# dimfeld/perceive

Hardware: AMD Instinct MI355X
Metric: vectors scanned/sec (exact cosine top-10, 384-d f32, batch=64) (higher is better)
Workload: dtype f32

## Files before the change

### include/perceive_hip.h

```cpp
#ifndef PERCEIVE_HIP_H
#define PERCEIVE_HIP_H

#include <stddef.h>
#include <stdint.h>

#ifdef __cplusplus
extern "C" {
#endif

typedef int pcv_status;
enum {
    PCV_OK = 0,
    PCV_ERR_INVALID = 1,
    PCV_ERR_DEVICE = 2,
    PCV_ERR_UNSUPPORTED = 3,
    PCV_ERR_IO = 4,
    PCV_ERR_INTERNAL = 5
};

enum { PCV_METRIC_COSINE = 0, PCV_METRIC_DOT = 1 };

typedef struct pcv_ctx pcv_ctx;
typedef struct pcv_searcher pcv_searcher;
typedef struct pcv_model pcv_model;
// ... 125 lines not shown
pcv_status pcv_comm_destroy(pcv_comm* c);
pcv_status pcv_searcher_search_sharded(pcv_searcher* s, pcv_comm* c, const float* queries, int n_queries,
                                       const int64_t* source_ids, int n_sources, int k, int64_t* out_ids,
                                       float* out_scores, int* out_counts);
pcv_status pcv_searcher_search_sharded_dq(pcv_searcher* s, pcv_comm* c, const void* d_queries, int n_queries,
                                          const int64_t* source_ids, int n_sources, int k, int64_t* out_ids,
                                          float* out_scores, int* out_counts);
pcv_status pcv_comm_all_gather(pcv_comm* c, const void* d_send, void* d_recv, size_t bytes_per_rank);

pcv_status pcv_dot_product(pcv_ctx* ctx, const float* a, int B, const float* m, int64_t N, int dim,
                           float* out);
pcv_status pcv_cosine_similarity(pcv_ctx* ctx, const float* a, int B, const float* m, int64_t N, int dim,
                                 float* out);

typedef struct pcv_scan_stats {
    int64_t rows_scanned;
    int64_t bytes_algorithmic;
    float scan_ms;
    float total_ms;
    int64_t candidates;
    int32_t scan_launches;
    int32_t overflow_reruns;
    int32_t kernel_used;
    int32_t screening_copy;
    float host_enqueue_ms;
    float host_wait_ms;
    int64_t bytes_streamed;
    int32_t speculation_reruns;
    int32_t mid_copy;
    int64_t coarse_survivors;
    int64_t mid_survivors;
    int64_t narrow_survivors;
    int32_t screen_bits;
} pcv_scan_stats;
pcv_status pcv_searcher_last_stats(pcv_searcher* s, pcv_scan_stats* out);


typedef struct pcv_model_desc {
    int32_t vocab_size;
    int32_t hidden;
    int32_t layers;
    int32_t heads;
    int32_t intermediate;
    int32_t max_positions;
    int32_t type_vocab;
    float layer_norm_eps;
    int32_t pooling;
    int32_t normalize;
    int32_t dense_out;
    int32_t dense_activation;
    int32_t max_seq_length;
    int32_t compute;
    int32_t embedding_size;
    int32_t shared_layers;
    int32_t hidden_act;
} pcv_model_desc;
enum { PCV_GELU_ERF = 0, PCV_GELU_TANH = 1 };
enum { PCV_POOL_MEAN = 0, PCV_POOL_CLS = 1, PCV_POOL_MAX = 2, PCV_POOL_MEAN_SQRT_LEN = 3 };
enum { PCV_ACT_IDENTITY = 0, PCV_ACT_TANH = 1 };
enum { PCV_COMPUTE_F32 = 0, PCV_COMPUTE_BF16X3 = 1, PCV_COMPUTE_F16X2 = 2 };

void pcv_model_desc_minilm_l6(pcv_model_desc* d);

pcv_status pcv_model_create(pcv_ctx* ctx, const pcv_model_desc* desc, const char* weights_path,
                            uint64_t synthetic_seed, pcv_model** out);
pcv_status pcv_model_destroy(pcv_model* m);
// ... 57 lines not shown
```

### perceive_amd/_ffi.py

```python
import ctypes as C
import os

_HERE = os.path.dirname(os.path.abspath(__file__))
LIB_PATH = os.path.join(_HERE, "libperceive_hip.so")

PCV_OK = 0
METRIC_COSINE, METRIC_DOT = 0, 1
KERNEL_AUTO, KERNEL_WAVE, KERNEL_MFMA = 0, 1, 2
POOL_MEAN, POOL_CLS, POOL_MAX, POOL_MEAN_SQRT_LEN = 0, 1, 2, 3
ACT_IDENTITY, ACT_TANH = 0, 1
COMPUTE_F32, COMPUTE_BF16X3, COMPUTE_F16X2 = 0, 1, 2


class PcvError(RuntimeError):
    def __init__(self, status, message):
        super().__init__(f"perceive_hip status {status}: {message}")
        self.status = status


class Hit(C.Structure):
    _fields_ = [("score", C.c_double), ("pos", C.c_int64), ("id", C.c_int64)]


class ScanStats(C.Structure):
    _fields_ = [
        ("rows_scanned", C.c_int64),
        ("bytes_algorithmic", C.c_int64),
        ("scan_ms", C.c_float),
        ("total_ms", C.c_float),
        ("candidates", C.c_int64),
        ("scan_launches", C.c_int32),
        ("overflow_reruns", C.c_int32),
        ("kernel_used", C.c_int32),
        ("screening_copy", C.c_int32),
        ("host_enqueue_ms", C.c_float),
        ("host_wait_ms", C.c_float),
        ("bytes_streamed", C.c_int64),
        ("speculation_reruns", C.c_int32),
        ("mid_copy", C.c_int32),
        ("coarse_survivors", C.c_int64),
        ("mid_survivors", C.c_int64),
        ("narrow_survivors", C.c_int64),
        ("screen_bits", C.c_int32),
    ]


class ModelDesc(C.Structure):
    _fields_ = [
        ("vocab_size", C.c_int32),
        ("hidden", C.c_int32),
        ("layers", C.c_int32),
        ("heads", C.c_int32),
        ("intermediate", C.c_int32),
        ("max_positions", C.c_int32),
        ("type_vocab", C.c_int32),
        ("layer_norm_eps", C.c_float),
        ("pooling", C.c_int32),
        ("normalize", C.c_int32),
        ("dense_out", C.c_int32),
        ("dense_activation", C.c_int32),
        ("max_seq_length", C.c_int32),
        ("compute", C.c_int32),
        ("embedding_size", C.c_int32),
        ("shared_layers", C.c_int32),
        ("hidden_act", C.c_int32),
    ]


class EncodeStats(C.Structure):
    _fields_ = [("total_ms", C.c_float), ("flops", C.c_double), ("batch", C.c_int32), ("seq_len", C.c_int32)]


_P = C.c_void_p
_I64P = C.c_void_p
_F32P = C.c_void_p
_U8P = C.c_void_p
# ... 145 lines not shown
```

### perceive_amd/csrc/scan.h

```cpp
#pragma once
#include <hip/hip_runtime.h>
#include <stdint.h>

#include "../../include/perceive_hip.h"

namespace pcv {

constexpr int kBlockRows = 32;
constexpr int kMaxK = PCV_MAX_RESULTS;
constexpr int kSeedPartRows = 256;
constexpr int kSeedParts = 64;
constexpr int kMaxWaveQueries = 4;
constexpr int kHot = 256;
constexpr int kMfmaQueries = 256;
constexpr int kScale8Stride = 1;

struct SegDesc {
    const float4* blk;
    const float* scale;
    const int64_t* ids;
    int64_t id0;
    int64_t pos0;
    uint32_t nrows;
    uint32_t nblocks;
    uint32_t blk0;
    uint32_t pad;
    const uint4* blk16;
    const uint4* blk8;
    const uint4* mid16;
    const float* scale16;
    const float* scale8;
    const uint4* blk6;
    const float4* scale6;
};
constexpr uint32_t kFlagSix = 1u << 31;
constexpr uint32_t kTuneNoSix = 1u << 29;
constexpr uint32_t kTuneForceSix = 1u << 31;

struct pcv_hit_dev {
    double score;
    int64_t pos;
    int64_t id;
};

struct CeilRec {
    double score;
    int64_t pos;
    float lo, hi;
};

struct ScanParams {
    const SegDesc* seg;
    int nseg;
    uint32_t total_blocks;
    int D;
    int D4;
    int B;
    int k;
    int metric;
    uint32_t tile_rows;
    const CeilRec* ceil;
    const float* queries;
    float* qf32;
    uint16_t* qbf16;
    int8_t* q8;
    float* q8c;
    float* qraw;
    float* margin;
    float* margin32;
    uint32_t* tau;
// ... 105 lines not shown
```

### perceive_amd/csrc/scan_kernels.hip

```cpp
#include <algorithm>
#include <cstdlib>
#include <numeric>
#include <type_traits>

#include "common.h"
#include "scan.h"
#include "synth.h"

#ifndef PCV_EXP
#define PCV_EXP 0
#endif
namespace pcv {
namespace {

typedef __bf16 bf16x8 __attribute__((ext_vector_type(8)));
typedef float f32x8 __attribute__((ext_vector_type(8)));
typedef float f32x16 __attribute__((ext_vector_type(16)));
typedef float f32x4 __attribute__((ext_vector_type(4)));

#define PCV_GLOBAL __attribute__((address_space(1)))
template <class T>
__device__ __forceinline__ T gld(const T* p) {
    return *(const PCV_GLOBAL T*)p;
}
// ... 304 lines not shown
        const float s_blk = !any_row ? __builtin_nanf("") : (bm > 0.0f ? 127.0f / bm : 1.0f);
        for (int g = h; g < D16; g += 2) {
            uint32_t w[4] = {0, 0, 0, 0};
#pragma unroll
            for (int e = 0; e < 4; ++e)
                if (searchable && 4 * g + e < D4) {
                    const float4 v = src[(size_t)(4 * g + e) * 32];
                    const float y[4] = {v.x * sc, v.y * sc, v.z * sc, v.w * sc};
#pragma unroll
                    for (int j = 0; j < 4; ++j) {
                        const int qv = max(-127, min(127, (int)rintf(y[j] * s_blk)));
                        w[e] |= (uint32_t)(qv & 0xff) << (8 * j);
                    }
                }
            blk8[((size_t)b * D16 + g) * 32 + r] = make_uint4(w[0], w[1], w[2], w[3]);
        }
        if (lane == 0) scale8[b] = s_blk;
    }
}


__global__ __launch_bounds__(256) void pack6_kernel(const float4* __restrict__ blk, const float* __restrict__ scale,
                                                    const uint4* __restrict__ blk8, const float* __restrict__ scale8,
                                                    const uint32_t* __restrict__ blocks, uint4* __restrict__ blk6,
                                                    float4* __restrict__ scale6, uint32_t first_block, uint32_t nblocks, int D4) {
    const int lane = threadIdx.x & 63, r = lane & 31, h = lane >> 5;
    const int D16 = ((D4 * 4 + 127) & ~127) >> 4, NCH = D16 >> 3;
    for (uint32_t i = (blocks ? 0u : first_block) + blockIdx.x * 4 + (threadIdx.x >> 6); i < nblocks; i += gridDim.x * 4) {
        const uint32_t b = blocks ? blocks[i] : i;
        const float sc = scale[(size_t)b * 32 + r];
        const float s = scale8[b];
        const bool searchable = sc != 0.0f && s == s;
        const double inv_s = searchable ? 1.0 / (double)s : 0.0;
        double e2 = 0.0, n2 = 0.0;
        for (int ch = 0; ch < NCH; ++ch) {
            uint32_t w[16];
#pragma unroll
            for (int ks = 0; ks < 4; ++ks) {
                const int f16 = ch * 8 + 2 * ks + h;
                const uint4 v = blk8[((size_t)b * D16 + f16) * 32 + r];
                w[4 * ks] = v.x;
                w[4 * ks + 1] = v.y;
                w[4 * ks + 2] = v.z;
                w[4 * ks + 3] = v.w;
#pragma unroll
                for (int e = 0; e < 4; ++e) {
                    const int f4 = 4 * f16 + e;
                    if (!searchable || f4 >= D4) continue;
                    const float4 x = blk[((size_t)b * D4 + f4) * 32 + r];
                    const float y[4] = {x.x * sc, x.y * sc, x.z * sc, x.w * sc};
                    const uint32_t word = w[4 * ks + e];
#pragma unroll
                    for (int j = 0; j < 4; ++j) {
                        const int x8 = (int)(int8_t)(word >> (8 * j));
                        const double xt = (double)(4 * (x8 >> 2)) * inv_s + 1.5 * inv_s;
                        const double d = (double)y[j] - xt;
                        e2 += d * d;
                        n2 += xt * xt;
                    }
                }
            }
            uint32_t u[16];
#pragma unroll
            for (int d = 0; d < 16; ++d) {
                const uint32_t biased = w[d] ^ 0x80808080u;
                u[d] = (biased >> 2) & 0x3f3f3f3fu;
            }
            uint32_t lo[8], hi[4];
#pragma unroll
            for (int k = 0; k < 8; ++k) lo[k] = (u[2 * k] & 0x0f0f0f0fu) | ((u[2 * k + 1] & 0x0f0f0f0fu) << 4);
#pragma unroll
            for (int k = 0; k < 4; ++k) {
                hi[k] = 0;
#pragma unroll
                for (int m = 0; m < 4; ++m) hi[k] |= ((u[4 * k + m] >> 4) & 0x03030303u) << (2 * m);
            }
            uint4* dst = blk6 + ((size_t)b * NCH + ch) * 3 * 64 + lane;
            dst[0] = make_uint4(lo[0], lo[1], lo[2], lo[3]);
            dst[64] = make_uint4(lo[4], lo[5], lo[6], lo[7]);
            dst[128] = make_uint4(hi[0], hi[1], hi[2], hi[3]);
        }
        e2 += __shfl_xor(e2, 32);
        n2 += __shfl_xor(n2, 32);
#pragma unroll
        for (int off = 16; off > 0; off >>= 1) {
            e2 = fmax(e2, __shfl_xor(e2, off));
            n2 = fmax(n2, __shfl_xor(n2, off));
        }
        if (lane == 0) {
            const float up = 1.0f + 0x1p-19f;
            const bool any = s == s;
            scale6[b] = make_float4(s, any ? (float)(sqrt(e2) * (double)s) * up : 0.0f, any ? (float)(sqrt(n2) * (double)s) * up : 0.0f, 0.0f);
        }
    }
}


__global__ __launch_bounds__(256) void mid_pack_kernel(const float4* __restrict__ blk, const float* __restrict__ scale, uint4* __restrict__ mid16,
                                                       float* __restrict__ scale16, uint32_t first_row, uint32_t nrows, int D4) {
    const int lane = threadIdx.x & 63;
    const int P8 = D4 >> 1;
    for (uint32_t row = first_row + blockIdx.x * 4 + (threadIdx.x >> 6); row < nrows; row += gridDim.x * 4) {
        const float sc = scale[row];
        const float4* src = blk + (size_t)(row >> 5) * D4 * 32 + (row & 31);
        float mx = 0.0f;
        for (int j = lane; j < P8; j += 64) {
            const float4 a = src[(size_t)(2 * j) * 32], b = src[(size_t)(2 * j + 1) * 32];
            mx = fmaxf(mx, fmaxf(fmaxf(fmaxf(fabsf(a.x * sc), fabsf(a.y * sc)), fmaxf(fabsf(a.z * sc), fabsf(a.w * sc))),
                                 fmaxf(fmaxf(fabsf(b.x * sc), fabsf(b.y * sc)), fmaxf(fabsf(b.z * sc), fabsf(b.w * sc)))));
        }
#pragma unroll
        for (int off = 32; off > 0; off >>= 1) mx = fmaxf(mx, __shfl_xor(mx, off));
        const bool searchable = sc != 0.0f && mx < __builtin_inff();
        const float s2 = !searchable ? 0.0f : (mx > 0.0f ? 32766.0f / mx : 1.0f);
        for (int j = lane; j < P8; j += 64) {
            const float4 a = src[(size_t)(2 * j) * 32], b = src[(size_t)(2 * j + 1) * 32];
            const float y[8] = {a.x * sc, a.y * sc, a.z * sc, a.w * sc, b.x * sc, b.y * sc, b.z * sc, b.w * sc};
            uint32_t w[4];
#pragma unroll
            for (int e = 0; e < 4; ++e) {
                const int lo = searchable ? max(-32767, min(32767, (int)rintf(y[2 * e] * s2))) : 0;
                const int hi = searchable ? max(-32767, min(32767, (int)rintf(y[2 * e + 1] * s2))) : 0;
                w[e] = ((uint32_t)lo & 0xffffu) | ((uint32_t)hi << 16);
            }
            mid16[(size_t)row * P8 + j] = make_uint4(w[0], w[1], w[2], w[3]);
// ... 524 lines not shown
    const int64_t i = t / D4src;
    const int f4 = (int)(t % D4src);
    if (i >= n) return;
    const int64_t gp = pos[i];
    int s = -1;
    for (int j = 0; j < nseg; ++j)
        if (gp >= segs[j].pos0 && gp < segs[j].pos0 + (int64_t)segs[j].nrows) s = j;
    float4 v = make_float4(__builtin_nanf(""), __builtin_nanf(""), __builtin_nanf(""), __builtin_nanf(""));
    int64_t id = -1;
    if (s >= 0) {
        const uint32_t row = (uint32_t)(gp - segs[s].pos0);
        v = segs[s].blk[((size_t)(row >> 5) * D4 + f4) * 32 + (row & 31)];
        id = segs[s].ids ? segs[s].ids[row] : segs[s].id0 + row;
    }
    const float vv[4] = {v.x, v.y, v.z, v.w};
    for (int j = 0; j < 4; ++j)
        if (f4 * 4 + j < D) out_rows[i * D + f4 * 4 + j] = vv[j];
    if (f4 == 0 && out_ids) out_ids[i] = id;
}


__global__ __launch_bounds__(256) void reset_scan_state_kernel(uint32_t* __restrict__ tau, uint32_t* __restrict__ slots,
                                                               uint32_t* __restrict__ cand_cnt) {
    const int t = blockIdx.x * 256 + threadIdx.x;
    if (t < kMfmaQueries * kMaxK) slots[t] = kKeyNegInf;
    if (t < kMfmaQueries) {
        tau[t * kHot] = kKeyNegInf;
        tau[kMfmaQueries * kHot + t] = kKeyNegInf;
        cand_cnt[t * kHot] = 0;
        cand_cnt[t * kHot + 32] = 0;
        cand_cnt[t * kHot + 33] = 0;
        cand_cnt[t * kHot + 34] = 0;
    }
}

__device__ __forceinline__ bool is_seed_block(const ScanParams& p, int si, uint32_t lb) {
    return si == 0 && (lb & ((1u << p.seed_shift) - 1u)) == 0 && (lb >> p.seed_shift) < p.seed_blocks;
}

__device__ __forceinline__ uint32_t seed_threshold_key(const ScanParams& p, int q, int sub ) {
    uint32_t mn = 0xffffffffu;
    if (q < p.B)
        for (int j = sub; j < p.k; j += 4) mn = min(mn, ld_relaxed(&p.slots[(size_t)q * kMaxK + j]));
    mn = min(mn, (uint32_t)__shfl_xor(mn, 1));
    mn = min(mn, (uint32_t)__shfl_xor(mn, 2));
    return q < p.B ? mn : kKeyNegInf;
}

__global__ __launch_bounds__(256) void upload_kernel(const uint4* __restrict__ src_pinned, uint4* __restrict__ dst, uint32_t n16) {
    const uint32_t i = blockIdx.x * 256 + threadIdx.x;
    if (i < n16) dst[i] = src_pinned[i];
}

template <int QG>
__global__ __launch_bounds__(256) void prep_seed_kernel(const ScanParams* __restrict__ pp, const float4* __restrict__ seg0_blk,
                                                        const float* __restrict__ seg0_scale, uint32_t nseed) {
    const ScanParams& p = *pp;
    extern __shared__ __attribute__((aligned(16))) float smem[];
    const int Dp = p.D4 * 4, D = p.D;
    float* sq = smem;
    uint32_t* gmax = (uint32_t*)(smem + QG * Dp);
    const int part = blockIdx.x, q0 = blockIdx.y * QG, tid = threadIdx.x;
    const bool writer = part == 0;
    static_assert(kSeedPartRows == 256, "one seed row per thread");
    const uint32_t sr = part * kSeedPartRows + tid;
    const uint32_t row = (((sr >> 5) << p.seed_shift) << 5) | (sr & 31);
// ... 736 lines not shown
    float sblk[kRing];
    uint32_t tail, head, done, pad;
};
__device__ __forceinline__ uint32_t lds_ld(const uint32_t* p) { return __hip_atomic_load(p, __ATOMIC_RELAXED, __HIP_MEMORY_SCOPE_WORKGROUP); }
__device__ __forceinline__ void lds_st(uint32_t* p, uint32_t v) { __hip_atomic_store(p, v, __ATOMIC_RELAXED, __HIP_MEMORY_SCOPE_WORKGROUP); }
__device__ __forceinline__ uint32_t lds_add(uint32_t* p, uint32_t v) {
    return __hip_atomic_fetch_add(p, v, __ATOMIC_RELAXED, __HIP_MEMORY_SCOPE_WORKGROUP);
}
#define PCV_LDS_ORDER() asm volatile("" ::: "memory")

template <bool SIX = false>
__device__ __forceinline__ void ring_push(SurvRing& ring, uint32_t m, const i32x16& acc, float sblk, uint32_t q, uint32_t hh, uint32_t si,
                                          uint32_t elb, float off = 0.0f) {
    const uint32_t n = (uint32_t)__builtin_popcount(m);
    uint32_t pos = 0;
    if (m) pos = lds_add(&ring.tail, n);
    while (__any(m != 0 && (pos + n - 1u) - lds_ld(&ring.head) >= kRing)) __builtin_amdgcn_s_sleep(2);
    const uint32_t hib = 0x80000000u | (si << 13) | (q << 5) | (4u * hh);
#pragma unroll
    for (int i = 0; i < 16; ++i) {
        if (m & (1u << i)) {
            const uint32_t slot = pos & (kRing - 1);
            lds_st(&ring.lo[slot], elb);
            ring.acc[slot] = SIX ? __builtin_bit_cast(int, fmaf(4.0f, (float)acc[i], off)) : acc[i];
            ring.sblk[slot] = sblk;
            PCV_LDS_ORDER();
            lds_st(&ring.hi[slot], hib + (uint32_t)((i & 3) + 8 * (i >> 2)));
            ++pos;
        }
    }
}

constexpr uint32_t kStack = 2048;
struct DrainStack {
    uint32_t lo[kStack], hi[kStack];
    int acc[kStack];
    float sblk[kStack];
};
constexpr int kSixMaxDp8 = 384;
constexpr int kSixPieces = kSixMaxDp8 / 16 / 8;
template <int NQ, bool SIX = false>
__device__ __forceinline__ void drain_survivors(const ScanParams& p, SurvRing& ring, DrainStack& stk, const uint32_t* ltau0, const float* lsq,
                                                const float* lvq, float* lU, int lane, int D4, uint32_t streaming, unsigned long long* stamp,
                                                const uint4* lq8 = nullptr, int LDQ = 0, float* lT6 = nullptr) {
    static_assert(NQ <= 64, "one query per lane");
#ifdef PCV_STAMPS
#define PCV_DSTAMP(slot) if (stamp && lane == 0) stamp[slot] = __builtin_amdgcn_s_memrealtime();
#define PCV_DCOUNT(slot, n) if (stamp && lane == 0) stamp[slot] += (n);
#define PCV_DMAX(hi, lo_) if (stamp && lane == 0) { const unsigned long long o = stamp[2]; \
        stamp[2] = (max(o >> 32, (unsigned long long)(hi)) << 32) | max(o & 0xffffffffull, (unsigned long long)(lo_)); }
#else
#define PCV_DSTAMP(slot)
#define PCV_DCOUNT(slot, n)
#define PCV_DMAX(hi, lo_)
#endif
    PCV_DSTAMP(0)
#ifdef PCV_STAMPS
    const unsigned long long clk0 = __builtin_amdgcn_s_memtime();
#endif
    const int Dp = D4 * 4, Dp8 = (Dp + 127) & ~127;
    const uint32_t g = (uint32_t)lane >> 3;
    const int sub = lane & 7;
    const int ql = lane < NQ ? lane : NQ - 1;
    const float my_sq = lsq[ql], my_vq = lvq[ql];
    const uint32_t my_tau0 = ltau0[ql];
    const float my_e32 = ql < p.B ? 0.5f * gld(&p.margin32[ql]) : 0.0f;
    const float nrm = (p.metric == PCV_METRIC_DOT) ? p.max_norm : 1.0f;
    const float c1 = 0.5002f * sqrtf((float)Dp8) * nrm;
    const float dead = (p.metric == PCV_METRIC_DOT) ? -__builtin_inff() : __builtin_inff();
    uint32_t my_tau = ld_relaxed(&p.tau_c[ql]);
    uint32_t head = 0, sp = 0, idle = 0;
    int c_si = -1;
    const float4* c_blk = nullptr;
    const float* c_scale = nullptr;
    const uint4* c_mid = nullptr;
    const float* c_s16 = nullptr;
    __builtin_amdgcn_s_setprio(3);

    auto work = [&](bool on, uint32_t hi, uint32_t lo) {
#ifdef PCV_STAMPS
        const unsigned long long ts = __builtin_amdgcn_s_memrealtime();
#endif
        const int q = (int)((hi >> 5) & 0xffu), rib = (int)(hi & 31u), si = (int)((hi >> 13) & ((1u << kRingSegBits) - 1u));
        const uint32_t lb = lo, row = lb * 32u + (uint32_t)rib;
        if (on && si != c_si) {
            c_si = si;
            c_blk = gld(&p.seg[si].blk);
            c_scale = gld(&p.seg[si].scale);
            c_mid = gld(&p.seg[si].mid16);
            c_s16 = gld(&p.seg[si].scale16);
        }
        float sc = 0.0f, m32 = 0.0f, s2 = 1.0f, l1 = 0.0f, part = 0.0f;
        uint32_t tkey = kKeyNegInf;
        const bool has_mid = on && c_mid != nullptr;
        const float* qf = p.qf32 + (size_t)q * Dp;
        if (on) {
            sc = gld(&c_scale[row]);
// ... 102 lines not shown
            first = false;
            int src = -1;
#pragma unroll
            for (uint32_t j = 0; j < 8; ++j) {
                if (set) {
                    const int s0 = __builtin_ctzll(set);
                    set &= set - 1;
                    if (g == j) src = s0;
                }
            }
            const bool on = src >= 0;
            work(on, (uint32_t)__shfl((int)ehi, on ? src : 0), (uint32_t)__shfl((int)elo, on ? src : 0));
        }
    };

    for (;;) {
        refresh((idle & 7u) == 0);

        uint32_t tail = lds_ld(&ring.tail);
        bool over = false;
        if (tail == head) {
            over = lds_ld(&ring.done) == streaming;
            if (over) {
                PCV_LDS_ORDER();
                tail = lds_ld(&ring.tail);
            }
        }
        if (tail != head) {
            idle = 0;
            const uint32_t n = min(tail - head, 64u);
            bool have = (uint32_t)lane < n;
            uint32_t ehi = 0, elo = 0;
            int eacc = 0;
            float esb = 0.0f;
            if (have) {
                const uint32_t slot = (head + (uint32_t)lane) & (kRing - 1);
                do ehi = lds_ld(&ring.hi[slot]);
                while (!(ehi & 0x80000000u));
                PCV_LDS_ORDER();
                elo = lds_ld(&ring.lo[slot]);
                eacc = ring.acc[slot];
                esb = ring.sblk[slot];
                PCV_LDS_ORDER();
                lds_st(&ring.hi[slot], 0u);
            }
            head += n;
            PCV_LDS_ORDER();
            if (lane == 0) lds_st(&ring.head, head);
            const int eq = (int)((ehi >> 5) & 0xffu);
            if constexpr (SIX) {
                if (have) g_atomic_add(&p.cand_cnt[eq * kHot + 34], 1u);
                have = have && __builtin_bit_cast(float, eacc) >= esb * __shfl(myT6, eq);
                const int P16 = ((D4 * 4 + 127) & ~127) >> 4;
                unsigned long long set = __ballot(have);
                while (set) {
                    const unsigned long long taken_from = set;
                    int src = -1;
#pragma unroll
                    for (uint32_t j = 0; j < 8; ++j) {
                        if (set) {
                            const int s0 = __builtin_ctzll(set);
                            set &= set - 1;
                            if (g == j) src = s0;
                        }
                    }
                    const unsigned long long taken = taken_from & ~set;
                    const bool on = src >= 0;
                    const uint32_t hi8 = (uint32_t)__shfl((int)ehi, on ? src : 0), lb8 = (uint32_t)__shfl((int)elo, on ? src : 0);
                    const int q8q = (int)((hi8 >> 5) & 0xffu), rib = (int)(hi8 & 31u), si8 = (int)((hi8 >> 13) & ((1u << kRingSegBits) - 1u));
                    int part = 0;
                    float sb = 0.0f;
                    if (on) {
                        const uint4* b8 = gld(&p.seg[si8].blk8);
                        sb = gld(gld(&p.seg[si8].scale8) + lb8);
                        uint4 v[kSixPieces];
#pragma unroll
                        for (int j = 0; j < kSixPieces; ++j)
                            if (sub + 8 * j < P16) v[j] = __builtin_bit_cast(uint4, gld4((const float4*)b8 + ((size_t)lb8 * P16 + sub + 8 * j) * 32 + rib));
#pragma unroll
                        for (int j = 0; j < kSixPieces; ++j)
                            if (sub + 8 * j < P16) {
                                const uint4 qv = lq8[(size_t)q8q * LDQ + sub + 8 * j];
                                part = __builtin_amdgcn_sdot4((int)v[j].x, (int)qv.x, part, false);
                                part = __builtin_amdgcn_sdot4((int)v[j].y, (int)qv.y, part, false);
                                part = __builtin_amdgcn_sdot4((int)v[j].z, (int)qv.z, part, false);
                                part = __builtin_amdgcn_sdot4((int)v[j].w, (int)qv.w, part, false);
                            }
                    }
#pragma unroll
                    for (int off = 4; off > 0; off >>= 1) part += __shfl_xor(part, off);
                    const int rank = (int)__builtin_popcountll(taken & ((1ull << lane) - 1ull));
                    const int a8 = __shfl(part, 8 * rank);
                    const float s8 = __shfl(sb, 8 * rank);
                    if ((taken >> lane) & 1ull) {
                        eacc = a8;
                        esb = s8;
                    }
                }
            }
            const float U = __shfl(myU, eq), vq = __shfl(my_vq, eq), Tq = __shfl(myT, eq);
            const float rhs = fmaf(esb, U, -vq);
            const bool keep = have && (float)eacc >= rhs;
            const bool likely = keep && (float)eacc >= fmaf(0.25f, rhs, 0.75f * esb * Tq);
            if (SIX ? keep : have) g_atomic_add(&p.cand_cnt[eq * kHot + 32], 1u);
            const unsigned long long wait = __ballot(keep && !likely);
            const uint32_t nw = (uint32_t)__builtin_popcountll(wait);
            PCV_DCOUNT(4, n)
            PCV_DCOUNT(7, n - (uint32_t)__builtin_popcountll(__ballot(keep)))
            PCV_DMAX(tail - (head - n), sp + nw)
            if (sp + nw <= kStack) {
                if (keep && !likely) {
                    const uint32_t at = sp + (uint32_t)__builtin_popcountll(wait & ((1ull << lane) - 1ull));
                    stk.lo[at] = elo;
                    stk.hi[at] = ehi;
                    stk.acc[at] = eacc;
                    stk.sblk[at] = esb;
                }
                sp += nw;
                work_set(__ballot(likely), ehi, elo);
            } else {
                work_set(__ballot(keep), ehi, elo);
            }
        } else if (sp > 0) {
            idle = 0;
            const uint32_t n = min(sp, 8u);
            sp -= n;
            const bool have = g < n;
            const uint32_t at = sp + (have ? g : 0u);
            const uint32_t ehi = stk.hi[at], elo = stk.lo[at];
            const int eacc = stk.acc[at];
            const float esb = stk.sblk[at];
            const int eq = (int)((ehi >> 5) & 0xffu);
            const float U = __shfl(myU, eq), vq = __shfl(my_vq, eq);
            const bool keep = have && (float)eacc >= fmaf(esb, U, -vq);
            PCV_DCOUNT(7, n - (uint32_t)__builtin_popcountll(__ballot(keep && sub == 0)))
            if (__any(keep)) work(keep, ehi, elo);
        } else if (over) {
            break;
        } else {
            ++idle;
            __builtin_amdgcn_s_sleep(4);
        }
    }
    PCV_DSTAMP(3)
    PCV_DCOUNT(1, __builtin_amdgcn_s_memtime() - clk0)
#undef PCV_DSTAMP
#undef PCV_DCOUNT
#undef PCV_DMAX
}

#ifdef PCV_STAMPS
#define PCV_STAMP(slot)                                                                                            \
    if (p.stamps && lane == 0) p.stamps[(size_t)(blockIdx.x * WPB + wave) * 8 + (slot)] = __builtin_amdgcn_s_memrealtime();
#ifdef PCV_STAMPS_TIMELINE
#define PCV_COUNT(slot, n) \
    if ((slot) < 5 && p.stamps && lane == 0) p.stamps[(size_t)(blockIdx.x * WPB + wave) * 8 + (slot)] += (n);
#else
#define PCV_COUNT(slot, n) \
    if (p.stamps && lane == 0) p.stamps[(size_t)(blockIdx.x * WPB + wave) * 8 + (slot)] += (n);
#endif
#else
#define PCV_STAMP(slot)
#define PCV_COUNT(slot, n)
#endif
template <int NT, bool NTL, int WPB, int NBUF, bool DRAIN, int NCHT, bool SIX = false>
__global__ __launch_bounds__(WPB * 64, NT == 4 ? 2 : 3) void scan_mfma8_kernel(const ScanParams* __restrict__ pp) {
    static_assert(!SIX || (DRAIN && NCHT > 0), "the 6-bit screen exists in the DRAIN form with a known chunk count");
    const ScanParams& p = *pp;
    constexpr uint32_t SW = DRAIN ? WPB - 1 : WPB;
    constexpr bool ULDS = DRAIN;
    extern __shared__ uint4 lq8[];
    const int D4 = p.D4;
    const int Dp = D4 * 4;
    const int Dp8 = (Dp + 127) & ~127;
    const int P16 = NCHT ? NCHT * 8 : Dp8 >> 4;
    const int LDQ = P16 + 1;
    const int NCH = NCHT ? NCHT : Dp8 >> 7;
    __shared__ uint32_t ltau0[NT * 32];
    __shared__ float lsq[NT * 32], lvq[NT * 32];
    __shared__ uint32_t ring_words[DRAIN ? sizeof(SurvRing) / 4 : 4];
    SurvRing& ring = *(SurvRing*)ring_words;
    __shared__ uint32_t stack_words[DRAIN ? sizeof(DrainStack) / 4 : 4];
    DrainStack& stack = *(DrainStack*)stack_words;
    __shared__ float lU[NT * 32];
    __shared__ float lT6[SIX ? NT * 32 : 1];
    const int lane = threadIdx.x & 63;
    const uint32_t wave = __builtin_amdgcn_readfirstlane(threadIdx.x >> 6);
    PCV_STAMP(0)
    if constexpr (DRAIN) {
        for (uint32_t i = threadIdx.x; i < kRing; i += WPB * 64) ring.hi[i] = 0u;
        if (threadIdx.x < 4) (&ring.tail)[threadIdx.x] = 0u;
    }
    for (int i = threadIdx.x; i < NT * 32 * P16; i += WPB * 64) {
        const int q = i / P16, pc = i - q * P16;
        lq8[(size_t)q * LDQ + pc] = __builtin_bit_cast(uint4, gld4((const float4*)p.q8 + i));
    }
    for (int q = threadIdx.x; q < NT * 32; q += WPB * 64) {
        lsq[q] = gld(&p.q8c[4 * q]);
        lvq[q] = gld(&p.q8c[4 * q + 1]);
    }
    for (int q = threadIdx.x >> 2; q < NT * 32; q += WPB * 16) {
        const uint32_t key = seed_threshold_key(p, q, threadIdx.x & 3);
        if ((threadIdx.x & 3) == 0) ltau0[q] = key;
    }
    __syncthreads();
    const int c = lane & 31, h = lane >> 5;
    const float nrm = (p.metric == PCV_METRIC_DOT) ? p.max_norm : 1.0f;
    const float c1 = 0.5002f * sqrtf((float)Dp8) * nrm;
    const float dead_u = (p.metric == PCV_METRIC_DOT) ? -__builtin_inff() : __builtin_inff();
    auto u_of = [&](int q, uint32_t tau_key, float e32q) -> float {
        const float sqq = lsq[q];
        const float T = (key_f32(max(ltau0[q], tau_key)) - e32q) * sqq;
        return (q < p.B) ? (sqq != 0.0f ? (T - fabsf(T) * 2e-6f) - c1 : dead_u) : __builtin_inff();
    };
    if constexpr (ULDS) {
        for (int q = threadIdx.x; q < NT * 32; q += WPB * 64) {
// ... 672 lines not shown
    pcv_hit_dev* out = p.out + (size_t)q * p.k;
    pcv_hit_dev* outh = p.out_host ? p.out_host + (size_t)q * p.k : nullptr;
    auto put = [&](int j, const pcv_hit_dev& hit) {
        out[j] = hit;
        if (outh) outh[j] = hit;
    };
    for (uint32_t i = tid; i < nv; i += 256) {
        const int r = rank_of(i, nv);
        if (r < p.k) {
            const uint64_t e = c_e[i];
            const SegDesc& sg = p.seg[(int)(e >> 32)];
            const uint32_t row = (uint32_t)e;
            pcv_hit_dev hit;
            hit.score = c_s[i];
            hit.pos = c_p[i];
            hit.id = sg.ids ? sg.ids[row] : sg.id0 + (int64_t)row;
            put(r, hit);
            if (r == p.k - 1 && p.kth_host) p.kth_host[q] = (float)c_s[i];
        }
    }
    if (tid == 0 && nv < (uint32_t)p.k && p.kth_host) p.kth_host[q] = __builtin_nanf("");
    pcv_hit_dev none;
    none.score = __builtin_nan("");
    none.pos = -1;
    none.id = -1;
    for (int j = (int)nv + tid; j < p.k; j += 256) put(j, none);
    if (tid == 0) {
        const bool failed = guessed && n_spec < (uint32_t)p.k;
        if (p.cnt_host) p.cnt_host[q] = failed ? kSpecFailed : raw_cnt;
        if (p.coarse_host) {
            p.coarse_host[q] = ld_relaxed(&p.cand_cnt[q * kHot + 32]);
            p.coarse_host[kMfmaQueries + q] = ld_relaxed(&p.cand_cnt[q * kHot + 33]);
            p.coarse_host[2 * kMfmaQueries + q] = ld_relaxed(&p.cand_cnt[q * kHot + 34]);
        }
        st_relaxed(&p.cand_cnt[q * kHot + 32], 0u);
        st_relaxed(&p.cand_cnt[q * kHot + 33], 0u);
        st_relaxed(&p.cand_cnt[q * kHot + 34], 0u);
        if ((raw_cnt > p.cand_cap || failed) && p.flag_rec) p.flag_rec->pos = 1;
        st_relaxed(&p.tau[q * kHot], kKeyNegInf);
        st_relaxed(&p.tau_c[q], kKeyNegInf);
        st_relaxed(&p.cand_cnt[q * kHot], 0u);
    }
    for (int j = tid; j < p.k; j += 256) st_relaxed(&p.slots[(size_t)q * kMaxK + j], kKeyNegInf);
}

__global__ __launch_bounds__(64) void merge_kernel(const pcv_hit_dev* __restrict__ lists_all, int n_shards, int B, int k,
                                                   size_t stride, int flagged, pcv_hit_dev* __restrict__ out) {
    extern __shared__ unsigned char taken[];
    const int q = blockIdx.x, lane = threadIdx.x;
    const int total = n_shards * k;
    if (flagged && q == 0 && lane == 0) {
        int64_t any = 0;
        for (int sh = 0; sh < n_shards; ++sh) any |= lists_all[sh * stride + (size_t)B * k].pos;
        pcv_hit_dev f;
        f.score = 0.0;
        f.pos = any ? 1 : 0;
        f.id = 0;
        out[(size_t)B * k] = f;
    }
    for (int i = lane; i < total; i += 64) taken[i] = 0;
    __syncthreads();
    for (int j = 0; j < k; ++j) {
        double bs = 0;
        int64_t bp = 0;
        int bi = -1;
        for (int i = lane; i < total; i += 64) {
            if (taken[i]) continue;
            const pcv_hit_dev& e = lists_all[(size_t)(i / k) * stride + (size_t)q * k + (i % k)];
            if (e.pos < 0 || !(e.score == e.score)) continue;
            if (bi < 0 || better(e.score, e.pos, bs, bp)) {
// ... 541 lines not shown
```

### perceive_amd/csrc/searcher.cpp

```cpp
#include <dlfcn.h>

#include <algorithm>
#include <chrono>
#include <cmath>
#include <cstdlib>
#include <cstring>
#include <iterator>
#include <memory>
#include <atomic>
#include <mutex>
#include <numeric>
#include <thread>
#include <vector>

#include "common.h"
#include "scan.h"

using namespace pcv;

namespace {

struct Segment {
    float4* blk = nullptr;
    float* scale = nullptr;
// ... 119 lines not shown
                m2 /= 2.0;
            }
            n += 1;
            const double dl = d - mean;
            mean += dl / (double)n;
            m2 += dl * (d - mean);
            spread += (sp - spread) / (double)n;
            smallest = std::min(smallest, d);
        }
        void reset() {
            n = 0;
            mean = m2 = spread = 0.0;
            smallest = INFINITY;
        }
        float gap() const {
            if (n < 128 || holdoff > 0) return NAN;
            const double sd = std::sqrt(m2 / (double)(n - 1));
            if (!(mean > 0.0) || sd > 0.15 * mean) return NAN;
            const double g = std::min(mean - 6.0 * sd, 0.8 * (double)smallest);
            return g > 0.0 ? (float)g : NAN;
        }
    } gaps;
    int64_t gap_rows = -1;
    int gap_k = 0, gap_nseg = 0;
    DevBuf<float> d_cand_s;
    DevBuf<uint32_t> d_tau, d_slots, d_cnt;
    DevBuf<uint64_t> d_cand;
    DevBuf<pcv_hit_dev> d_hits;
    uint8_t* pin_pass = nullptr;
    uint8_t* d_pass = nullptr;
    size_t pass_cap = 0;
    struct Pinned {
        uint32_t cnt[kMfmaQueries];
        uint32_t coarse[3 * kMfmaQueries];
        float spec_base[kMfmaQueries];
        float spec_top[kMfmaQueries];
        float kth[kMfmaQueries];
        pcv_hit_dev hits[kMfmaQueries * kMaxK];
    };
    Pinned* pin = nullptr;
    bool state_clean = false;
    uint32_t cand_cap = 8192;
    uint32_t scan_flags = 0;
    bool fail_copy_alloc = false;
    int mid_copy = PCV_MID_COPY_AUTO;
    bool mid_gave_way = false;
    bool mids_present = false;
    int mid_hot_passes = 0;
    hipStream_t side = nullptr;
    hipEvent_t side_go = nullptr, mid_done = nullptr;
    bool mid_building = false;
    struct MidTask {
        struct Item {
            Segment* g;
            const float4* blk;
            const float* scale;
            const float* scale8;
            uint32_t cap_rows, first_row, rows;
            uint4* mid16;
            float* scale16;
            bool own;
        };
        std::vector<Item> items;
        std::thread th;
        std::atomic<bool> queued{false};
        bool joined = false, failed = false;
    };
// ... 1095 lines not shown
    p.seg = reinterpret_cast<const SegDesc*>(s->d_pass + L.off_seg);
    p.nseg = nseg;
    p.total_blocks = blk0;
    p.D = s->D;
    p.D4 = s->D4;
    p.B = B;
    p.k = k;
    p.metric = s->metric;
    p.tile_rows = kernel == PCV_KERNEL_MFMA ? mfma_tile_rows(B) : 0u;
    p.queries = reinterpret_cast<const float*>(s->d_pass + L.off_q);
    if (ceil_host) {
        std::memcpy(s->pin_pass + L.off_ceil, ceil_host, (size_t)B * sizeof(CeilRec));
        p.ceil = reinterpret_cast<const CeilRec*>(s->d_pass + L.off_ceil);
    }
    p.qf32 = s->d_qf32.p;
    p.qbf16 = s->d_qbf16.p;
    p.q8 = s->d_q8.p;
    p.q8c = s->d_q8c.p;
    p.qraw = s->d_qraw.p;
    p.margin = s->d_margin.p;
    p.margin32 = s->d_margin32.p;
    p.tau = s->d_tau.p;
    p.tau_c = s->d_tau.p + (size_t)kMfmaQueries * kHot;
    p.slots = s->d_slots.p;
    p.cand_cnt = s->d_cnt.p;
    p.cand = s->d_cand.p;
    p.cand_s = s->d_cand_s.p;
    p.out = d_out ? d_out : s->d_hits.p;
    p.out_host = download ? s->pin->hits : nullptr;
    p.cnt_host = s->pin->cnt;
    p.coarse_host = s->pin->coarse;
    p.flag_rec = d_flag;
    p.cand_cap = s->cand_cap;
    p.flags = (s->scan_flags & ~(16u | 64u | kFlagSix)) | (src_kind == 1 ? 16u : 0u) | (src_kind == 2 ? 64u : 0u);
    const bool six = src_kind == 2 && have_six && nseg > 0 && s->kernel == PCV_KERNEL_AUTO && !(s->scan_flags & kTuneNoSix) &&
                     mfma8_six_pass(B, s->Dp, p.flags, nseg);
    if (six) p.flags |= kFlagSix;
    const uint32_t seed_parts = ((s->scan_flags >> 16) & 0xff) ? ((s->scan_flags >> 16) & 0xff) : kSeedParts;
    p.seed_blocks = std::min<uint32_t>(std::min<uint32_t>(seed_parts, kSeedParts) * kSeedPartRows / kBlockRows, segs[0].g->nblocks());
    p.seed_shift = 0;
    while (((uint64_t)p.seed_blocks << (p.seed_shift + 1)) <= segs[0].g->nblocks() && p.seed_shift < 20) ++p.seed_shift;
    p.spec = s->d_spec.p;
    p.spec_rank = 0;
    p.spec_gap = NAN;
    p.spec_spread = 0.0f;
    p.spec_base_host = s->pin->spec_base;
    p.spec_top_host = s->pin->spec_top;
    p.kth_host = s->pin->kth;
    if (s->gap_rows != rows || s->gap_k != k || s->gap_nseg != nseg) {
        s->gap_rows = rows;
        s->gap_k = k;
        s->gap_nseg = nseg;
        s->gaps.reset();
    }
    if (kernel == PCV_KERNEL_MFMA && !s->spec_hold && s->spec_rest == 0 && !(s->scan_flags & 32u) && k >= 2 && !ceil_host) {
        if (!(s->scan_flags & 128u)) p.spec_gap = s->gaps.gap();
        p.spec_spread = (float)s->gaps.spread;
        const double r = (double)std::min<int64_t>(tab[0].nrows, (int64_t)p.seed_blocks * kBlockRows) / (double)std::max<int64_t>(rows, 1);
        double binom = 1.0, rj = 1.0;
        for (int j = 1; j < k && r < 0.25; ++j) {
            binom *= (double)(k - j) / (double)j;
            rj *= r;
            if (binom * rj < 1e-6) {
                p.spec_rank = j;
                break;
            }
        }
// ... 137 lines not shown
        ms_scan = ms_total * s->graph_fixed_ms;
    } else {
        (void)hipEventElapsedTime(&ms_scan, s->ev[1], s->ev[2]);
        s->shape_fixed_ms = ms_total > 0.0f ? std::min(1.0f, std::max(0.0f, ms_scan / ms_total)) : 0.0f;
    }
    s->stats.scan_ms += ms_scan;
    s->stats.total_ms += ms_total;
    s->stats.scan_launches += 1;
    s->stats.rows_scanned += rows;
    s->stats.bytes_algorithmic += rows * (int64_t)s->D * 4;
    s->stats.bytes_streamed += s->pending.stream_bytes;
    s->stats.screening_copy = s->pending.src;
    s->stats.screen_bits = s->pending.src == 2 ? (s->pending.six ? 6 : 8) : 0;

    const uint32_t* cnt = s->pin->cnt;
    uint32_t mx = 0;
    int64_t sum = 0;
    bool guess_failed = false;
    for (int b = 0; b < B; ++b) {
        if (cnt[b] == kSpecFailed) {
            guess_failed = true;
            continue;
        }
        mx = std::max(mx, cnt[b]);
        sum += cnt[b];
    }
    int64_t coarse = 0;
    for (int b = 0; b < B; ++b) {
        coarse += s->pin->coarse[b];
        s->stats.mid_survivors += s->pin->coarse[kMfmaQueries + b];
        if (s->pending.six) s->stats.narrow_survivors += s->pin->coarse[2 * kMfmaQueries + b];
    }
    s->stats.coarse_survivors += coarse;
    s->stats.mid_copy = s->pending.mid ? 1 : 0;
    const int64_t fine_bytes = coarse * (int64_t)s->Dp * 32;
    if (s->pending.src == 2 && !s->pending.mid &&
        (coarse > kMidTrigger * (int64_t)B || fine_bytes * kMidShare > (int64_t)s->pending.int8_bytes))
        s->mid_hot_passes += 1;
    else
        s->mid_hot_passes = 0;
    if (mx <= s->cand_cap && !guess_failed) {
        s->stats.candidates += sum;
        s->spec_hold = false;
        if (s->spec_rest > 0) s->spec_rest -= 1;
        if (s->spec_penalty > 0 && ++s->spec_clean >= 4096) s->spec_penalty = s->spec_clean = 0;
        if (s->pending.guessing) {
            for (int b = 0; b < B; ++b) {
                const float d = s->pin->kth[b] - s->pin->spec_base[b];
                const float sp = s->pin->spec_top[b] - s->pin->spec_base[b];
                if (d == d && std::isfinite(d) && sp == sp && std::isfinite(sp)) s->gaps.add(d, sp);
            }
        }
        if (s->gaps.holdoff > 0) s->gaps.holdoff -= 1;
        return false;
    }
    if (guess_failed) {
        s->stats.speculation_reruns += 1;
        s->spec_hold = true;
        if (s->pending.learned) {
            s->gaps.reset();
            s->gaps.holdoff = 256;
        } else {
            s->spec_penalty = std::min(1024, s->spec_penalty ? 2 * s->spec_penalty : 16);
            s->spec_rest = s->spec_penalty;
            s->spec_clean = 0;
        }
// ... 1205 lines not shown
        if (c->pin_cap < n + 1) {
            if (c->pin_hits) (void)hipHostFree(c->pin_hits);
            c->pin_hits = nullptr;
            c->pin_cap = 0;
            PCV_HIP(hipHostMalloc((void**)&c->pin_hits, (n + 1) * sizeof(pcv_hit_dev), hipHostMallocDefault));
            c->pin_cap = n + 1;
        }
        auto exchange = [&](const pcv_hit_dev* local, size_t nq, int flagged) {
            const size_t rec = nq * k + flagged;
            rccl_check(rccl().AllGather(local, c->d_gathered.p, rec * sizeof(pcv_hit_dev),  0, c->comm, st),
                       "ncclAllGather");
            launch_merge(st, c->d_gathered.p, c->world, (int)nq, k, c->d_merged.p, flagged);
            PCV_HIP(hipMemcpyAsync(c->pin_hits, c->d_merged.p, rec * sizeof(pcv_hit_dev), hipMemcpyDeviceToHost, st));
        };
        const int qstep = pass_queries(s, pick_kernel(s, n_queries), true);
        std::vector<pcv_hit_dev> all(n);
        pcv_scan_stats total{};
        auto accumulate = [&] {
            total.rows_scanned += s->stats.rows_scanned;
            total.bytes_algorithmic += s->stats.bytes_algorithmic;
            total.scan_ms += s->stats.scan_ms;
            total.total_ms += s->stats.total_ms;
            total.candidates += s->stats.candidates;
            total.scan_launches += s->stats.scan_launches;
            total.overflow_reruns += s->stats.overflow_reruns;
            total.speculation_reruns += s->stats.speculation_reruns;
            total.host_enqueue_ms += s->stats.host_enqueue_ms;
            total.host_wait_ms += s->stats.host_wait_ms;
            total.kernel_used = s->stats.kernel_used;
            total.bytes_streamed += s->stats.bytes_streamed;
            total.coarse_survivors += s->stats.coarse_survivors;
            total.mid_survivors += s->stats.mid_survivors;
            total.narrow_survivors += s->stats.narrow_survivors;
            total.mid_copy = s->stats.mid_copy;
            total.screening_copy = s->stats.screening_copy;
            total.screen_bits = s->stats.screen_bits;
        };
        for (int q0 = 0; q0 < n_queries; q0 += qstep) {
            const int B = std::min(qstep, n_queries - q0);
            const size_t nb = (size_t)B * k;
            for (int attempt = 0;; ++attempt) {
                device_begin(s, queries + (size_t)q0 * s->D, B, source_ids, n_sources, k, c->d_local.p, queries_on_device);
                try {
                    exchange(c->d_local.p, (size_t)B, 1);
                } catch (...) {
                    try {
                        finish_pass(s);
                    } catch (...) {
                    }
                    throw;
                }
                finish_pass(s);
                const bool again = c->pin_hits[nb].pos != 0;
                if (!again) std::memcpy(all.data() + (size_t)q0 * k, c->pin_hits, nb * sizeof(pcv_hit_dev));
                accumulate();
                if (!again) break;
                s->spec_hold = true;
                PCV_REQUIRE(attempt < 7,
                            "search_sharded: the step is still incomplete on some rank after %d repeats (on this rank: %d candidate-list "
                            "overflows, %d speculative thresholds that did not hold)",
                            attempt + 1, total.overflow_reruns, total.speculation_reruns);
            }
        }
        s->stats = total;
        hits_to_outputs(s->metric, s->D, all.data(), n_queries, k, out_ids, out_scores, out_counts);
    });
// ... 51 lines not shown
```

### shim/perceive-core/src/ffi.rs

```rust
#![allow(non_camel_case_types, dead_code)]
use std::os::raw::{c_char, c_int, c_void};

#[repr(C)]
pub struct pcv_ctx {
    _private: [u8; 0],
}
#[repr(C)]
pub struct pcv_searcher {
    _private: [u8; 0],
}
#[repr(C)]
pub struct pcv_model {
    _private: [u8; 0],
}
#[repr(C)]
pub struct pcv_tokenizer {
    _private: [u8; 0],
}
#[repr(C)]
pub struct pcv_comm {
    _private: [u8; 0],
}

#[repr(C)]
#[derive(Debug, Clone, Copy, Default)]
pub struct pcv_hit {
    pub score: f64,
    pub pos: i64,
    pub id: i64,
}

#[repr(C)]
#[derive(Debug, Clone, Copy, Default)]
pub struct pcv_scan_stats {
    pub rows_scanned: i64,
    pub bytes_algorithmic: i64,
    pub scan_ms: f32,
    pub total_ms: f32,
    pub candidates: i64,
    pub scan_launches: i32,
    pub overflow_reruns: i32,
    pub kernel_used: i32,
    pub screening_copy: i32,
    pub host_enqueue_ms: f32,
    pub host_wait_ms: f32,
    pub bytes_streamed: i64,
    pub speculation_reruns: i32,
    pub mid_copy: i32,
    pub coarse_survivors: i64,
    pub mid_survivors: i64,
    pub narrow_survivors: i64,
    pub screen_bits: i32,
}

#[repr(C)]
#[derive(Debug, Clone, Copy, Default)]
pub struct pcv_model_desc {
    pub vocab_size: i32,
    pub hidden: i32,
    pub layers: i32,
    pub heads: i32,
    pub intermediate: i32,
    pub max_positions: i32,
    pub type_vocab: i32,
    pub layer_norm_eps: f32,
    pub pooling: i32,
    pub normalize: i32,
    pub dense_out: i32,
    pub dense_activation: i32,
    pub max_seq_length: i32,
    pub compute: i32,
    pub embedding_size: i32,
    pub shared_layers: i32,
    pub hidden_act: i32,
}

#[repr(C)]
#[derive(Debug, Clone, Copy, Default)]
pub struct pcv_encode_stats {
    pub total_ms: f32,
    pub flops: f64,
    pub batch: i32,
    pub seq_len: i32,
}

// ... 141 lines not shown
```

Measured before the change: 20.86 billion.

## Add optional L2-style tighter bound to six-bit survivor screening

Extends the six-bit packing to store a per-block int8 residual norm, and adds an opt-in tighter pruning bound in the survivor drain that uses query error terms and a per-candidate t2 value kept in the drain stack. It also adds a six_survivors counter with a global atomic per ballot and exposes it through stats. The tighter bound is gated behind a tuning flag that is off by default, so the default path only gains the extra counter atomic, the scale6 loads in place of scale8, and a slightly larger shared stack.

```diff
diff --git a/include/perceive_hip.h b/include/perceive_hip.h
--- a/include/perceive_hip.h
+++ b/include/perceive_hip.h
@@ -181,6 +181,7 @@
     int64_t mid_survivors;
     int64_t narrow_survivors;
     int32_t screen_bits;
+    int64_t six_survivors;
 } pcv_scan_stats;
 pcv_status pcv_searcher_last_stats(pcv_searcher* s, pcv_scan_stats* out);
 
diff --git a/perceive_amd/_ffi.py b/perceive_amd/_ffi.py
--- a/perceive_amd/_ffi.py
+++ b/perceive_amd/_ffi.py
@@ -42,6 +42,7 @@
         ("mid_survivors", C.c_int64),
         ("narrow_survivors", C.c_int64),
         ("screen_bits", C.c_int32),
+        ("six_survivors", C.c_int64),
     ]
 
 
diff --git a/perceive_amd/csrc/scan.h b/perceive_amd/csrc/scan.h
--- a/perceive_amd/csrc/scan.h
+++ b/perceive_amd/csrc/scan.h
@@ -36,6 +36,8 @@
 constexpr uint32_t kFlagSix = 1u << 31;
 constexpr uint32_t kTuneNoSix = 1u << 29;
 constexpr uint32_t kTuneForceSix = 1u << 31;
+constexpr uint32_t kTuneSixL2 = 1u << 6;
+constexpr uint32_t kFlagSixL2 = 1u << 30;
 
 struct pcv_hit_dev {
     double score;
diff --git a/perceive_amd/csrc/scan_kernels.hip b/perceive_amd/csrc/scan_kernels.hip
--- a/perceive_amd/csrc/scan_kernels.hip
+++ b/perceive_amd/csrc/scan_kernels.hip
@@ -360,7 +360,7 @@
         const float s = scale8[b];
         const bool searchable = sc != 0.0f && s == s;
         const double inv_s = searchable ? 1.0 / (double)s : 0.0;
-        double e2 = 0.0, n2 = 0.0;
+        double e2 = 0.0, n2 = 0.0, e8 = 0.0;
         for (int ch = 0; ch < NCH; ++ch) {
             uint32_t w[16];
 #pragma unroll
@@ -382,9 +382,10 @@
                     for (int j = 0; j < 4; ++j) {
                         const int x8 = (int)(int8_t)(word >> (8 * j));
                         const double xt = (double)(4 * (x8 >> 2)) * inv_s + 1.5 * inv_s;
-                        const double d = (double)y[j] - xt;
+                        const double d = (double)y[j] - xt, d8 = (double)y[j] - (double)x8 * inv_s;
                         e2 += d * d;
                         n2 += xt * xt;
+                        e8 += d8 * d8;
                     }
                 }
             }
@@ -410,15 +411,18 @@
         }
         e2 += __shfl_xor(e2, 32);
         n2 += __shfl_xor(n2, 32);
+        e8 += __shfl_xor(e8, 32);
 #pragma unroll
         for (int off = 16; off > 0; off >>= 1) {
             e2 = fmax(e2, __shfl_xor(e2, off));
             n2 = fmax(n2, __shfl_xor(n2, off));
+            e8 = fmax(e8, __shfl_xor(e8, off));
         }
         if (lane == 0) {
             const float up = 1.0f + 0x1p-19f;
             const bool any = s == s;
-            scale6[b] = make_float4(s, any ? (float)(sqrt(e2) * (double)s) * up : 0.0f, any ? (float)(sqrt(n2) * (double)s) * up : 0.0f, 0.0f);
+            scale6[b] = make_float4(s, any ? (float)(sqrt(e2) * (double)s) * up : 0.0f, any ? (float)(sqrt(n2) * (double)s) * up : 0.0f,
+                                    any ? (float)(sqrt(e8) * (double)s) * up : 0.0f);
         }
     }
 }
@@ -1009,6 +1013,7 @@
         cand_cnt[t * kHot + 33] = 0;
         cand_cnt[t * kHot + 34] = 0;
     }
+    if (t == 0) cand_cnt[35] = 0;
 }
 
 __device__ __forceinline__ bool is_seed_block(const ScanParams& p, int si, uint32_t lb) {
@@ -1811,15 +1816,17 @@
 }
 
 constexpr uint32_t kStack = 2048;
+template <bool SIX>
 struct DrainStack {
     uint32_t lo[kStack], hi[kStack];
     int acc[kStack];
     float sblk[kStack];
+    float t2[SIX ? kStack : 1];
 };
 constexpr int kSixMaxDp8 = 384;
 constexpr int kSixPieces = kSixMaxDp8 / 16 / 8;
 template <int NQ, bool SIX = false>
-__device__ __forceinline__ void drain_survivors(const ScanParams& p, SurvRing& ring, DrainStack& stk, const uint32_t* ltau0, const float* lsq,
+__device__ __forceinline__ void drain_survivors(const ScanParams& p, SurvRing& ring, DrainStack<SIX>& stk, const uint32_t* ltau0, const float* lsq,
                                                 const float* lvq, float* lU, int lane, int D4, uint32_t streaming, unsigned long long* stamp,
                                                 const uint4* lq8 = nullptr, int LDQ = 0, float* lT6 = nullptr) {
     static_assert(NQ <= 64, "one query per lane");
@@ -1842,6 +1849,13 @@
     const int sub = lane & 7;
     const int ql = lane < NQ ? lane : NQ - 1;
     const float my_sq = lsq[ql], my_vq = lvq[ql];
+    const bool l2 = SIX && (p.flags & kFlagSixL2) != 0;
+    const float my_a6 = SIX ? gld(&p.q8c[4 * kMfmaQueries + 4 * ql]) : 0.0f, my_e6 = SIX ? gld(&p.q8c[4 * kMfmaQueries + 4 * ql + 1]) : 0.0f;
+    const float n8_extra = 1.5f * sqrtf((float)Dp);
+    auto rhs_l2 = [](float sb, float T6, float t2, int acc) -> float {
+        const float st = sb * T6;
+        return (st - t2) - 0x1p-21f * (fabsf(st) + t2 + fabsf((float)acc));
+    };
     const uint32_t my_tau0 = ltau0[ql];
     const float my_e32 = ql < p.B ? 0.5f * gld(&p.margin32[ql]) : 0.0f;
     const float nrm = (p.metric == PCV_METRIC_DOT) ? p.max_norm : 1.0f;
@@ -2010,7 +2024,7 @@
             bool have = (uint32_t)lane < n;
             uint32_t ehi = 0, elo = 0;
             int eacc = 0;
-            float esb = 0.0f;
+            float esb = 0.0f, et2 = 0.0f;
             if (have) {
                 const uint32_t slot = (head + (uint32_t)lane) & (kRing - 1);
                 do ehi = lds_ld(&ring.hi[slot]);
@@ -2031,6 +2045,7 @@
                 have = have && __builtin_bit_cast(float, eacc) >= esb * __shfl(myT6, eq);
                 const int P16 = ((D4 * 4 + 127) & ~127) >> 4;
                 unsigned long long set = __ballot(have);
+                if (set && lane == 0) g_atomic_add(&p.cand_cnt[35], (uint32_t)__builtin_popcountll(set));
                 while (set) {
                     const unsigned long long taken_from = set;
                     int src = -1;
@@ -2047,10 +2062,10 @@
                     const uint32_t hi8 = (uint32_t)__shfl((int)ehi, on ? src : 0), lb8 = (uint32_t)__shfl((int)elo, on ? src : 0);
                     const int q8q = (int)((hi8 >> 5) & 0xffu), rib = (int)(hi8 & 31u), si8 = (int)((hi8 >> 13) & ((1u << kRingSegBits) - 1u));
                     int part = 0;
-                    float sb = 0.0f;
+                    float4 s6 = make_float4(0.0f, 0.0f, 0.0f, 0.0f);
                     if (on) {
                         const uint4* b8 = gld(&p.seg[si8].blk8);
-                        sb = gld(gld(&p.seg[si8].scale8) + lb8);
+                        s6 = gld4(gld(&p.seg[si8].scale6) + lb8);
                         uint4 v[kSixPieces];
 #pragma unroll
                         for (int j = 0; j < kSixPieces; ++j)
@@ -2068,17 +2083,26 @@
 #pragma unroll
                     for (int off = 4; off > 0; off >>= 1) part += __shfl_xor(part, off);
                     const int rank = (int)__builtin_popcountll(taken & ((1ull << lane) - 1ull));
+                    const float t2g = fmaf(s6.w, __shfl(my_a6, q8q), (s6.z + n8_extra) * __shfl(my_e6, q8q)) * (1.0f + 0x1p-20f);
                     const int a8 = __shfl(part, 8 * rank);
-                    const float s8 = __shfl(sb, 8 * rank);
+                    const float s8 = __shfl(s6.x, 8 * rank), t8 = __shfl(t2g, 8 * rank);
                     if ((taken >> lane) & 1ull) {
                         eacc = a8;
                         esb = s8;
+                        et2 = t8;
                     }
                 }
             }
             const float U = __shfl(myU, eq), vq = __shfl(my_vq, eq), Tq = __shfl(myT, eq);
-            const float rhs = fmaf(esb, U, -vq);
-            const bool keep = have && (float)eacc >= rhs;
+            float rhs = fmaf(esb, U, -vq);
+            bool keep = have && (float)eacc >= rhs;
+            if constexpr (SIX) {
+                if (l2) {
+                    const float r2 = rhs_l2(esb, __shfl(myT6, eq), et2, eacc);
+                    keep = keep && (float)eacc >= r2;
+                    rhs = fmaxf(rhs, r2);
+                }
+            }
             const bool likely = keep && (float)eacc >= fmaf(0.25f, rhs, 0.75f * esb * Tq);
             if (SIX ? keep : have) g_atomic_add(&p.cand_cnt[eq * kHot + 32], 1u);
             const unsigned long long wait = __ballot(keep && !likely);
@@ -2093,6 +2117,7 @@
                     stk.hi[at] = ehi;
                     stk.acc[at] = eacc;
                     stk.sblk[at] = esb;
+                    if constexpr (SIX) stk.t2[at] = et2;
                 }
                 sp += nw;
                 work_set(__ballot(likely), ehi, elo);
@@ -2110,7 +2135,11 @@
             const float esb = stk.sblk[at];
             const int eq = (int)((ehi >> 5) & 0xffu);
             const float U = __shfl(myU, eq), vq = __shfl(my_vq, eq);
-            const bool keep = have && (float)eacc >= fmaf(esb, U, -vq);
+            bool keep = have && (float)eacc >= fmaf(esb, U, -vq);
+            if constexpr (SIX) {
+                const float T6 = __shfl(myT6, eq);
+                if (l2) keep = keep && (float)eacc >= rhs_l2(esb, T6, stk.t2[at], eacc);
+            }
             PCV_DCOUNT(7, n - (uint32_t)__builtin_popcountll(__ballot(keep && sub == 0)))
             if (__any(keep)) work(keep, ehi, elo);
         } else if (over) {
@@ -2158,8 +2187,8 @@
     __shared__ float lsq[NT * 32], lvq[NT * 32];
     __shared__ uint32_t ring_words[DRAIN ? sizeof(SurvRing) / 4 : 4];
     SurvRing& ring = *(SurvRing*)ring_words;
-    __shared__ uint32_t stack_words[DRAIN ? sizeof(DrainStack) / 4 : 4];
-    DrainStack& stack = *(DrainStack*)stack_words;
+    __shared__ uint32_t stack_words[DRAIN ? sizeof(DrainStack<SIX>) / 4 : 4];
+    DrainStack<SIX>& stack = *(DrainStack<SIX>*)stack_words;
     __shared__ float lU[NT * 32];
     __shared__ float lT6[SIX ? NT * 32 : 1];
     const int lane = threadIdx.x & 63;
@@ -2898,10 +2927,12 @@
             p.coarse_host[q] = ld_relaxed(&p.cand_cnt[q * kHot + 32]);
             p.coarse_host[kMfmaQueries + q] = ld_relaxed(&p.cand_cnt[q * kHot + 33]);
             p.coarse_host[2 * kMfmaQueries + q] = ld_relaxed(&p.cand_cnt[q * kHot + 34]);
+            if (q == 0) p.coarse_host[3 * kMfmaQueries] = ld_relaxed(&p.cand_cnt[35]);
         }
         st_relaxed(&p.cand_cnt[q * kHot + 32], 0u);
         st_relaxed(&p.cand_cnt[q * kHot + 33], 0u);
         st_relaxed(&p.cand_cnt[q * kHot + 34], 0u);
+        if (q == 0) st_relaxed(&p.cand_cnt[35], 0u);
         if ((raw_cnt > p.cand_cap || failed) && p.flag_rec) p.flag_rec->pos = 1;
         st_relaxed(&p.tau[q * kHot], kKeyNegInf);
         st_relaxed(&p.tau_c[q], kKeyNegInf);
diff --git a/perceive_amd/csrc/searcher.cpp b/perceive_amd/csrc/searcher.cpp
--- a/perceive_amd/csrc/searcher.cpp
+++ b/perceive_amd/csrc/searcher.cpp
@@ -175,7 +175,7 @@
     size_t pass_cap = 0;
     struct Pinned {
         uint32_t cnt[kMfmaQueries];
-        uint32_t coarse[3 * kMfmaQueries];
+        uint32_t coarse[3 * kMfmaQueries + 1];
         float spec_base[kMfmaQueries];
         float spec_top[kMfmaQueries];
         float kth[kMfmaQueries];
@@ -1337,7 +1337,8 @@
     p.coarse_host = s->pin->coarse;
     p.flag_rec = d_flag;
     p.cand_cap = s->cand_cap;
-    p.flags = (s->scan_flags & ~(16u | 64u | kFlagSix)) | (src_kind == 1 ? 16u : 0u) | (src_kind == 2 ? 64u : 0u);
+    p.flags = (s->scan_flags & ~(16u | 64u | kFlagSix | kFlagSixL2)) | (src_kind == 1 ? 16u : 0u) | (src_kind == 2 ? 64u : 0u);
+    if (s->scan_flags & kTuneSixL2) p.flags |= kFlagSixL2;
     const bool six = src_kind == 2 && have_six && nseg > 0 && s->kernel == PCV_KERNEL_AUTO && !(s->scan_flags & kTuneNoSix) &&
                      mfma8_six_pass(B, s->Dp, p.flags, nseg);
     if (six) p.flags |= kFlagSix;
@@ -1541,6 +1542,7 @@
         if (s->pending.six) s->stats.narrow_survivors += s->pin->coarse[2 * kMfmaQueries + b];
     }
     s->stats.coarse_survivors += coarse;
+    if (s->pending.six) s->stats.six_survivors += s->pin->coarse[3 * kMfmaQueries];
     s->stats.mid_copy = s->pending.mid ? 1 : 0;
     const int64_t fine_bytes = coarse * (int64_t)s->Dp * 32;
     if (s->pending.src == 2 && !s->pending.mid &&
@@ -2812,6 +2814,7 @@
             total.coarse_survivors += s->stats.coarse_survivors;
             total.mid_survivors += s->stats.mid_survivors;
             total.narrow_survivors += s->stats.narrow_survivors;
+            total.six_survivors += s->stats.six_survivors;
             total.mid_copy = s->stats.mid_copy;
             total.screening_copy = s->stats.screening_copy;
             total.screen_bits = s->stats.screen_bits;
diff --git a/shim/perceive-core/src/ffi.rs b/shim/perceive-core/src/ffi.rs
--- a/shim/perceive-core/src/ffi.rs
+++ b/shim/perceive-core/src/ffi.rs
@@ -51,6 +51,7 @@
     pub mid_survivors: i64,
     pub narrow_survivors: i64,
     pub screen_bits: i32,
+    pub six_survivors: i64,
 }
 
 #[repr(C)]
```

Result: slower. 17.82 billion (-14.6%).
